# viniciusvidal2/slam-sensor-fusion

Hardware: AMD Instinct MI355X
Metric: scans_per_s_200k_scan_vs_10M_map (higher is better)
Workload: dtype f32 points / f64 accumulation

## Files before the change

slam_sensor_fusion_amd/csrc/sf_nn.hpp:

```cpp
#pragma once
#include "sf_common.hpp"

namespace sf {

#ifdef SF_PHASE_TRACE
constexpr int PH_SLOTS = 16, PH_SHARDS = 64;
struct PhaseClock {
    unsigned long long t;
    unsigned acc[PH_SLOTS];
    __device__ __forceinline__ void start() { for (int i = 0; i < PH_SLOTS; ++i) acc[i] = 0; t = __builtin_amdgcn_s_memtime(); }
    __device__ __forceinline__ void mark(int i) { const unsigned long long n = __builtin_amdgcn_s_memtime(); acc[i] += (unsigned)(n - t); t = n; }
    __device__ __forceinline__ void count(int i, unsigned v) { acc[i] += v; }
};
#define SF_PH(pc, i) do { if (pc) (pc)->mark(i); } while (0)
#define SF_PHC(pc, i, v) do { if (pc) (pc)->count(i, v); } while (0)
#else
struct PhaseClock {};
#define SF_PH(pc, i) do { } while (0)
#define SF_PHC(pc, i, v) do { } while (0)
#endif

struct NNHit {
    float d2;
    int j;
    float px, py, pz;
    float lb2;
};

__device__ __forceinline__ float l2_simple(float qx, float qy, float qz, float px, float py, float pz)
{
    float dx = qx - px, dy = qy - py, dz = qz - pz;
    float r = __fmul_rn(dx, dx);
    r = __fadd_rn(r, __fmul_rn(dy, dy));
    r = __fadd_rn(r, __fmul_rn(dz, dz));
    return r;
}

__device__ __forceinline__ bool window_accepts(const SfWindow &w, float px, float py, float pz)
{
    if (w.kind == 1) return l2_simple(w.c[0], w.c[1], w.c[2], px, py, pz) < w.r2;
    if (w.kind == 2) {
        double d0 = (double)px - w.oc[0], d1 = (double)py - w.oc[1], d2 = (double)pz - w.oc[2];
        bool ok = true;
#pragma unroll
        for (int k = 0; k < 3; ++k) {
            double proj = __dadd_rn(__dadd_rn(__dmul_rn(d0, w.oR[k]), __dmul_rn(d1, w.oR[3 + k])), __dmul_rn(d2, w.oR[6 + k]));
            ok = ok && (fabs(proj) <= w.ohalf[k]);
        }
        return ok;
    }
    return true;
}

__device__ __forceinline__ float window_gap(const SfWindow &w, float qx, float qy, float qz)
{
    if (w.kind == 1) {
        const float dx = qx - w.c[0], dy = qy - w.c[1], dz = qz - w.c[2];
        return fmaxf(sqrtf(dx * dx + dy * dy + dz * dz) * 0.9995f - sqrtf(w.r2) * 1.0005f - 1.0e-4f, 0.0f);
    }
    if (w.kind == 2) {
        const double d0 = (double)qx - w.oc[0], d1 = (double)qy - w.oc[1], d2 = (double)qz - w.oc[2];
        double out = 0.0;
#pragma unroll
        for (int k = 0; k < 3; ++k) {
            const double proj = d0 * w.oR[k] + d1 * w.oR[3 + k] + d2 * w.oR[6 + k];
            const double n2 = w.oR[k] * w.oR[k] + w.oR[3 + k] * w.oR[3 + k] + w.oR[6 + k] * w.oR[6 + k];
            const double over = fmax(fabs(proj) - w.ohalf[k], 0.0);
            out = fmax(out, over / sqrt(fmax(n2, 1.0e-30)));
        }
        return fmaxf((float)out * 0.9995f - 1.0e-4f, 0.0f);
    }
    return 0.0f;
}

__device__ __forceinline__ unsigned long long hit_key(float d2, int j) { return ((unsigned long long)__float_as_uint(d2) << 32) | (unsigned long long)(uint32_t)j; }

__device__ __forceinline__ float search_start(float thr) { return thr > 0.0f ? __uint_as_float(__float_as_uint(thr) - 1u) : -1.0f; }

template <bool WINDOW, bool TRACK = false>
__device__ __forceinline__ void consider(const SfWindow &w, float px, float py, float pz, int j, bool valid, float qx, float qy, float qz, NNHit &hit)
{
    const float d2 = l2_simple(qx, qy, qz, px, py, pz);
    const bool take = valid && hit_key(d2, j) < hit_key(hit.d2, hit.j) && (!WINDOW || window_accepts(w, px, py, pz));
    if (TRACK) hit.lb2 = __builtin_amdgcn_fmed3f((valid && j != hit.j) ? d2 : 3.0e38f, hit.d2, hit.lb2);
    if (take) {
        hit.d2 = d2;
        hit.j = j;
        hit.px = px; hit.py = py; hit.pz = pz;
    }
}

#ifndef SF_NN_CLAMPED_LOADS
__device__ __forceinline__ float4 load_point(const SfGrid &g, uint32_t j, bool valid)
{
    typedef unsigned int u4 __attribute__((ext_vector_type(4)));
    const __amdgpu_buffer_rsrc_t rsrc = __builtin_amdgcn_make_buffer_rsrc((void *)g.pts, 0, (int)((uint32_t)g.n * 16u), 0x00020000);
    const u4 v = __builtin_amdgcn_raw_buffer_load_b128(rsrc, valid ? (int)(j * 16u) : -1, 0, 0);
    return make_float4(__uint_as_float(v.x), __uint_as_float(v.y), __uint_as_float(v.z), __uint_as_float(v.w));
}
#endif

template <bool WINDOW, bool TRACK = false>
__device__ __forceinline__ void scan4(const SfGrid &g, const SfWindow &w, uint32_t j, uint32_t b, float qx, float qy, float qz, NNHit &hit)
{
#ifndef SF_NN_CLAMPED_LOADS
    const float4 p0 = load_point(g, j, true), p1 = load_point(g, j + 1, j + 1 < b), p2 = load_point(g, j + 2, j + 2 < b), p3 = load_point(g, j + 3, j + 3 < b);
    consider<WINDOW, TRACK>(w, p0.x, p0.y, p0.z, (int)j, true, qx, qy, qz, hit);
    consider<WINDOW, TRACK>(w, p1.x, p1.y, p1.z, (int)(j + 1), j + 1 < b, qx, qy, qz, hit);
    consider<WINDOW, TRACK>(w, p2.x, p2.y, p2.z, (int)(j + 2), j + 2 < b, qx, qy, qz, hit);
    consider<WINDOW, TRACK>(w, p3.x, p3.y, p3.z, (int)(j + 3), j + 3 < b, qx, qy, qz, hit);
#else
    const uint32_t last = b - 1;
    const uint32_t j1 = min(j + 1, last), j2 = min(j + 2, last), j3 = min(j + 3, last);
    const float4 p0 = g.pts[j], p1 = g.pts[j1], p2 = g.pts[j2], p3 = g.pts[j3];
    consider<WINDOW, TRACK>(w, p0.x, p0.y, p0.z, (int)j, true, qx, qy, qz, hit);
    consider<WINDOW, TRACK>(w, p1.x, p1.y, p1.z, (int)j1, j + 1 < b, qx, qy, qz, hit);
    consider<WINDOW, TRACK>(w, p2.x, p2.y, p2.z, (int)j2, j + 2 < b, qx, qy, qz, hit);
    consider<WINDOW, TRACK>(w, p3.x, p3.y, p3.z, (int)j3, j + 3 < b, qx, qy, qz, hit);
#endif
}

template <bool WINDOW, bool TRACK = false>
__device__ __forceinline__ void scan_range(const SfGrid &g, const SfWindow &w, uint32_t a, uint32_t b, float qx, float qy, float qz, NNHit &hit)
{
    for (uint32_t j = a; j < b; j += 4) scan4<WINDOW, TRACK>(g, w, j, b, qx, qy, qz, hit);
}

__device__ __forceinline__ float min3f(float a, float b, float c) { return fminf(fminf(a, b), c); }

struct __attribute__((packed, aligned(4))) RowBounds { uint32_t s0, s1, s2, s3; };
__device__ __forceinline__ RowBounds load_row_bounds(const SfGrid &g, size_t cell)
{
    return *reinterpret_cast<const RowBounds *>(g.cell_start + cell - 1);
}

template <bool WINDOW>
__device__ __forceinline__ void scan_row(const SfGrid &g, const SfWindow &w, const RowBounds &rb, float gap2yz, float gxm2, float gxp2, bool xm, bool xp, float qx,
                                         float qy, float qz, NNHit &hit)
{
    scan_range<WINDOW>(g, w, rb.s1, rb.s2, qx, qy, qz, hit);
    if (xm && (gap2yz + gxm2) * 0.998f < hit.d2) scan_range<WINDOW>(g, w, rb.s0, rb.s1, qx, qy, qz, hit);
    if (xp && (gap2yz + gxp2) * 0.998f < hit.d2) scan_range<WINDOW>(g, w, rb.s2, rb.s3, qx, qy, qz, hit);
}

__device__ __forceinline__ float safe_gap(float gap, float eps) { return fmaxf(gap - eps, 0.0f); }

__device__ __forceinline__ float cell_gap(float gc, int c, int cq)
{
    if (c == cq) return 0.0f;
    float d = c < cq ? gc - (float)(c + 1) : (float)c - gc;
    return d > 0.0f ? d : 0.0f;
}

template <bool WINDOW>
__device__ __forceinline__ void nn_rings(const SfGrid &g, const SfWindow &w, float qx, float qy, float qz, int R_first, NNHit &hit)
{
    const float gx = (qx - g.org[0]) * g.inv_h, gy = (qy - g.org[1]) * g.inv_h, gz = (qz - g.org[2]) * g.inv_h;
    const int nx = g.dim[0], ny = g.dim[1], nz = g.dim[2];
    const int cx = (int)fminf(fmaxf(floorf(gx), 0.0f), (float)(nx - 1));
    const int cy = (int)fminf(fmaxf(floorf(gy), 0.0f), (float)(ny - 1));
    const int cz = (int)fminf(fmaxf(floorf(gz), 0.0f), (float)(nz - 1));
    const float h = g.h;
    const int rcap = max(nx, max(ny, nz));

    for (int R = R_first; R <= rcap; ++R) {
        {
            const int x0 = max(cx - R, 0), x1 = min(cx + R, nx - 1);
            const int y0 = max(cy - R, 0), y1 = min(cy + R, ny - 1);
            const int z0 = max(cz - R, 0), z1 = min(cz + R, nz - 1);
            if (R == 1) {
                constexpr uint32_t OYP = 0u | (2u << 2) | (1u << 4) | (1u << 6) | (0u << 8) | (2u << 10) | (0u << 12) | (2u << 14);
                constexpr uint32_t OZP = 1u | (1u << 2) | (0u << 4) | (2u << 6) | (0u << 8) | (0u << 10) | (2u << 12) | (2u << 14);
                const float fx = gx - (float)cx, fy = gy - (float)cy, fz = gz - (float)cz;
                const float ge = g.gap_eps;
                const float gxm = safe_gap(fx * h, ge), gxp = safe_gap((1.0f - fx) * h, ge);
                const float gym = safe_gap(fy * h, ge), gyp = safe_gap((1.0f - fy) * h, ge);
                const float gzm = safe_gap(fz * h, ge), gzp = safe_gap((1.0f - fz) * h, ge);
                const float gxm2 = gxm * gxm, gxp2 = gxp * gxp;
                const bool xm = cx > 0, xp = cx < nx - 1;
                auto row_gap2 = [&](int k) -> float {
                    const int dy = (int)((OYP >> (2 * k)) & 3u) - 1, dz = (int)((OZP >> (2 * k)) & 3u) - 1;
                    const float ry = dy < 0 ? gym : (dy > 0 ? gyp : 0.0f);
                    const float rz = dz < 0 ? gzm : (dz > 0 ? gzp : 0.0f);
                    return ry * ry + rz * rz;
                };
                auto row_cell = [&](int k) -> size_t {
                    const int dy = (int)((OYP >> (2 * k)) & 3u) - 1, dz = (int)((OZP >> (2 * k)) & 3u) - 1;
                    return ((size_t)(cz + dz) * ny + (cy + dy)) * nx + cx;
                };
                {
                    const RowBounds rb = load_row_bounds(g, ((size_t)cz * ny + cy) * nx + cx);
                    scan_row<WINDOW>(g, w, rb, 0.0f, gxm2, gxp2, xm, xp, qx, qy, qz, hit);
                }
                uint32_t mask = 0;
#pragma unroll
                for (int k = 0; k < 8; ++k) {
                    const int dy = (int)((OYP >> (2 * k)) & 3u) - 1, dz = (int)((OZP >> (2 * k)) & 3u) - 1;
                    const bool inside = (unsigned)(cy + dy) < (unsigned)ny && (unsigned)(cz + dz) < (unsigned)nz;
                    if (inside && row_gap2(k) * 0.998f < hit.d2) mask |= 1u << k;
                }
                int k = -1;
                RowBounds cur = {0, 0, 0, 0};
                if (mask) {
                    k = __ffs((int)mask) - 1;
                    mask &= mask - 1;
                    cur = load_row_bounds(g, row_cell(k));
                }
                while (k >= 0) {
                    int k1 = -1;
                    RowBounds nxt = cur;
                    while (mask) {
                        const int kk = __ffs((int)mask) - 1;
                        mask &= mask - 1;
                        if (row_gap2(kk) * 0.998f < hit.d2) {
                            k1 = kk;
                            nxt = load_row_bounds(g, row_cell(kk));
                            break;
                        }
                    }
                    const float g2 = row_gap2(k);
                    if (g2 * 0.998f < hit.d2) scan_row<WINDOW>(g, w, cur, g2, gxm2, gxp2, xm, xp, qx, qy, qz, hit);
                    k = k1;
                    cur = nxt;
                }
            } else {
                for (int z = z0; z <= z1; ++z) {
                    const float rz = safe_gap(cell_gap(gz, z, cz) * h, g.gap_eps);
                    for (int y = y0; y <= y1; ++y) {
                        const float ry = safe_gap(cell_gap(gy, y, cy) * h, g.gap_eps);
                        if ((ry * ry + rz * rz) * 0.998f >= hit.d2) continue;
                        const size_t row = ((size_t)z * ny + y) * nx;
                        scan_range<WINDOW>(g, w, g.cell_start[row + x0], g.cell_start[row + x1 + 1], qx, qy, qz, hit);
                    }
                }
            }
        }
        float m = 3.0e38f;
        if (cx - R > 0) m = fminf(m, (gx - (float)(cx - R)) * h);
        if (cx + R < nx - 1) m = fminf(m, ((float)(cx + R + 1) - gx) * h);
        if (cy - R > 0) m = fminf(m, (gy - (float)(cy - R)) * h);
        if (cy + R < ny - 1) m = fminf(m, ((float)(cy + R + 1) - gy) * h);
        if (cz - R > 0) m = fminf(m, (gz - (float)(cz - R)) * h);
        if (cz + R < nz - 1) m = fminf(m, ((float)(cz + R + 1) - gz) * h);
        if (m >= 3.0e38f) break;
        const float mm = safe_gap(m, g.gap_eps) * 0.999f;
        if (hit.d2 <= mm * mm) break;
    }
}

template <bool WINDOW>
__device__ __forceinline__ NNHit nn_search(const SfGrid &g, const SfWindow &w, float qx, float qy, float qz, float thr)
{
    NNHit hit;
    hit.d2 = search_start(thr);
    hit.j = -1;
    hit.px = hit.py = hit.pz = 0.0f;
    hit.lb2 = 0.0f;
    if (!(isfinite(qx) && isfinite(qy) && isfinite(qz)) || g.n == 0) return hit;
    if (WINDOW) {
        const float gap = window_gap(w, qx, qy, qz);
        if (gap * gap > thr) return hit;
    }
    nn_rings<WINDOW>(g, w, qx, qy, qz, 1, hit);
    return hit;
}

struct WaveNN {
    unsigned long long best[64];
    uint32_t lb2[64];
    float4 q[64];
    RowBounds rb0[64];
    float gap[6][64];
    unsigned long long cell0[64];
    uint16_t task[64 * 11];
};

__device__ __forceinline__ unsigned long long pack_hit(float d2, int j) { return ((unsigned long long)__float_as_uint(d2) << 32) | (unsigned long long)(uint32_t)j; }

struct QueryGeo {
    int cx, cy, cz;
    float gxm2, gxp2;
    float gym, gyp, gzm, gzp;
};

__device__ __forceinline__ QueryGeo query_geo(const SfGrid &g, float qx, float qy, float qz)
{
    QueryGeo G;
    const float gx = (qx - g.org[0]) * g.inv_h, gy = (qy - g.org[1]) * g.inv_h, gz = (qz - g.org[2]) * g.inv_h;
    G.cx = (int)fminf(fmaxf(floorf(gx), 0.0f), (float)(g.dim[0] - 1));
    G.cy = (int)fminf(fmaxf(floorf(gy), 0.0f), (float)(g.dim[1] - 1));
    G.cz = (int)fminf(fmaxf(floorf(gz), 0.0f), (float)(g.dim[2] - 1));
    const float h = g.h;
    const float fx = gx - (float)G.cx, fy = gy - (float)G.cy, fz = gz - (float)G.cz;
    const float ge = g.gap_eps;
    const float gxm = safe_gap(fx * h, ge), gxp = safe_gap((1.0f - fx) * h, ge);
    G.gxm2 = G.cx > 0 ? gxm * gxm : 3.0e38f;
    G.gxp2 = G.cx < g.dim[0] - 1 ? gxp * gxp : 3.0e38f;
    G.gym = safe_gap(fy * h, ge);
    G.gyp = safe_gap((1.0f - fy) * h, ge);
    G.gzm = safe_gap(fz * h, ge);
    G.gzp = safe_gap((1.0f - fz) * h, ge);
    return G;
}

__device__ __forceinline__ int row_dy(int k) { return (int)((0x8858u >> (2 * k)) & 3u) - 1; }
__device__ __forceinline__ int row_dz(int k) { return (int)((0xa085u >> (2 * k)) & 3u) - 1; }

__device__ __forceinline__ float row_gap2(const QueryGeo &G, int k)
{
    const int dy = row_dy(k), dz = row_dz(k);
    const float ry = dy < 0 ? G.gym : (dy > 0 ? G.gyp : 0.0f);
    const float rz = dz < 0 ? G.gzm : (dz > 0 ? G.gzp : 0.0f);
    return ry * ry + rz * rz;
}

template <bool WINDOW, bool COOP = false>
__device__ __forceinline__ NNHit nn_search_wave(const SfGrid &g, const SfWindow &w, bool valid, float qx, float qy, float qz, float thr, WaveNN *ws, NNHit seed = NNHit{0.0f, -1, 0.0f, 0.0f, 0.0f, 0.0f},
                                               PhaseClock *pc = nullptr)
{
    const int lane = (int)__lane_id();
    const int nx = g.dim[0], ny = g.dim[1], nz = g.dim[2];
    NNHit hit;
    hit.d2 = search_start(thr);
    hit.j = -1;
    hit.px = hit.py = hit.pz = 0.0f;
    hit.lb2 = 3.0e38f;
    valid = valid && isfinite(qx) && isfinite(qy) && isfinite(qz) && g.n > 0;
    if (WINDOW && valid) {
        const float gap = window_gap(w, qx, qy, qz);
        if (gap * gap > thr) {
            hit.lb2 = gap * gap;
            valid = false;
        }
    }
    if (valid) {
        const float ox = fmaxf(fmaxf(g.org[0] - qx, qx - (g.org[0] + (float)nx * g.h)), 0.0f);
        const float oy = fmaxf(fmaxf(g.org[1] - qy, qy - (g.org[1] + (float)ny * g.h)), 0.0f);
        const float oz = fmaxf(fmaxf(g.org[2] - qz, qz - (g.org[2] + (float)nz * g.h)), 0.0f);
        const float gap = fmaxf(sqrtf(ox * ox + oy * oy + oz * oz) * 0.9995f - 1.0e-3f, 0.0f);
        if (gap * gap > thr) {
            hit.lb2 = gap * gap;
            valid = false;
        }
    }
    if (valid && seed.j >= 0 && seed.d2 < thr) { hit.d2 = seed.d2; hit.j = seed.j; hit.px = seed.px; hit.py = seed.py; hit.pz = seed.pz; }
    uint32_t mask = 0;
#ifdef SF_PHASE_TRACE
    QueryGeo G{};
    RowBounds rb0{0, 0, 0, 0};
    if (valid) {
        G = query_geo(g, qx, qy, qz);
        rb0 = load_row_bounds(g, ((size_t)G.cz * ny + G.cy) * nx + G.cx);
        ws->rb0[lane] = rb0;
    }
    SF_PH(pc, 1);
    if (valid && rb0.s1 < rb0.s2) scan4<WINDOW, true>(g, w, rb0.s1, rb0.s2, qx, qy, qz, hit);
    SF_PH(pc, 2);
    if (valid) {
#else
    if (valid) {
        const QueryGeo G = query_geo(g, qx, qy, qz);
        const RowBounds rb0 = load_row_bounds(g, ((size_t)G.cz * ny + G.cy) * nx + G.cx);
        ws->rb0[lane] = rb0;
        if (rb0.s1 < rb0.s2) scan4<WINDOW, true>(g, w, rb0.s1, rb0.s2, qx, qy, qz, hit);
#endif
        if (rb0.s1 + 4 < rb0.s2) {
            if (hit.d2 > 0.0f) mask |= 1u << 10;
            else hit.lb2 = 0.0f;
        }
        if (rb0.s0 < rb0.s1) {
            if (G.gxm2 * 0.998f < hit.d2) mask |= 1u;
            else hit.lb2 = fminf(hit.lb2, G.gxm2);
        }
        if (rb0.s2 < rb0.s3) {
            if (G.gxp2 * 0.998f < hit.d2) mask |= 2u;
            else hit.lb2 = fminf(hit.lb2, G.gxp2);
        }
#pragma unroll
        for (int k = 0; k < 8; ++k) {
            const bool inside = (unsigned)(G.cy + row_dy(k)) < (unsigned)ny && (unsigned)(G.cz + row_dz(k)) < (unsigned)nz;
            const float gap2 = row_gap2(G, k);
            if (inside) {
                if (gap2 * 0.998f < hit.d2) mask |= 4u << k;
                else hit.lb2 = fminf(hit.lb2, gap2);
            }
        }
        if (mask) {
            ws->gap[0][lane] = G.gxm2; ws->gap[1][lane] = G.gxp2;
            ws->gap[2][lane] = G.gym; ws->gap[3][lane] = G.gyp; ws->gap[4][lane] = G.gzm; ws->gap[5][lane] = G.gzp;
            ws->cell0[lane] = ((unsigned long long)G.cz * (unsigned long long)ny + (unsigned long long)G.cy) * (unsigned long long)nx + (unsigned long long)G.cx;
        }
    }
    ws->best[lane] = pack_hit(hit.d2, hit.j);
    ws->lb2[lane] = __float_as_uint(hit.lb2);
    ws->q[lane] = make_float4(qx, qy, qz, 0.0f);
    int total = 0;
#pragma unroll
    for (int t = 0; t < 11; ++t) {
        const bool has = (mask >> t) & 1u;
        const unsigned long long bal = __ballot(has);
        const int rank = (int)__builtin_amdgcn_mbcnt_hi((uint32_t)(bal >> 32), __builtin_amdgcn_mbcnt_lo((uint32_t)bal, 0u));
        if (has) ws->task[total + rank] = (uint16_t)((lane << 4) | t);
        total += __popcll(bal);
    }
    __builtin_amdgcn_fence(__ATOMIC_ACQ_REL, "wavefront");
    __builtin_amdgcn_wave_barrier();
    SF_PH(pc, 3);
    SF_PHC(pc, 11, (unsigned)total);
#ifdef SF_PHASE_TRACE
    unsigned lane_trips = 0, lane_cands = 0;
#endif
    for (int i0 = 0; i0 < total; i0 += 64) {
        SF_PHC(pc, 9, 1u);
        const int idx = i0 + lane;
#ifdef SF_PHASE_TRACE
        unsigned my_trips = 0;
#endif
        if (idx < total) {
            const uint32_t e = ws->task[idx];
            const int owner = (int)(e >> 4), t = (int)(e & 15u);
            const float4 Q = ws->q[owner];
            QueryGeo G;
            G.cx = G.cy = G.cz = 0;
            G.gxm2 = ws->gap[0][owner]; G.gxp2 = ws->gap[1][owner];
            G.gym = ws->gap[2][owner]; G.gyp = ws->gap[3][owner]; G.gzm = ws->gap[4][owner]; G.gzp = ws->gap[5][owner];
            const unsigned long long start = __atomic_load_n(&ws->best[owner], __ATOMIC_RELAXED);
            const float cur = __uint_as_float((uint32_t)(start >> 32));
            const bool own_row = t < 2 || t == 10;
            const float g2 = own_row ? (t == 0 ? G.gxm2 : (t == 1 ? G.gxp2 : 0.0f)) : row_gap2(G, t - 2);
            float bound = g2;
            if (g2 * 0.998f < cur) {
                uint32_t a, b;
                bound = 3.0e38f;
                if (own_row) {
                    const RowBounds rb = ws->rb0[owner];
                    a = t == 0 ? rb.s0 : (t == 1 ? rb.s2 : rb.s1 + 4);
                    b = t == 0 ? rb.s1 : (t == 1 ? rb.s3 : rb.s2);
                } else {
                    const long long step = ((long long)row_dz(t - 2) * ny + row_dy(t - 2)) * nx;
                    const RowBounds rb = load_row_bounds(g, (size_t)((long long)ws->cell0[owner] + step));
                    const bool xm = (g2 + G.gxm2) * 0.998f < cur, xp = (g2 + G.gxp2) * 0.998f < cur;
                    a = xm ? rb.s0 : rb.s1;
                    b = xp ? rb.s3 : rb.s2;
                    if (!xm && rb.s0 < rb.s1) bound = g2 + G.gxm2;
                    if (!xp && rb.s2 < rb.s3) bound = fminf(bound, g2 + G.gxp2);
                }
                NNHit h;
                h.d2 = cur;
                h.j = (int)(uint32_t)start;
                h.px = h.py = h.pz = 0.0f;
                h.lb2 = 3.0e38f;
                scan_range<WINDOW, true>(g, w, a, b, Q.x, Q.y, Q.z, h);
#ifdef SF_PHASE_TRACE
                my_trips = (b - a + 3u) / 4u; lane_cands += b - a; lane_trips += my_trips;
#endif
                bound = fminf(bound, h.lb2);
                const unsigned long long mine = pack_hit(h.d2, h.j);
                if (mine != start) {
                    const unsigned long long old = atomicMin(&ws->best[owner], mine);
                    bound = fminf(bound, __uint_as_float((uint32_t)((old > mine ? old : mine) >> 32)));
                }
            }
            atomicMin(&ws->lb2[owner], __float_as_uint(bound));
        }
#ifdef SF_PHASE_TRACE
        { unsigned m = my_trips; for (int o = 32; o > 0; o >>= 1) m = max(m, (unsigned)__shfl_xor((int)m, o)); SF_PHC(pc, 10, m); }
#endif
    }
    __builtin_amdgcn_fence(__ATOMIC_ACQ_REL, "wavefront");
    __builtin_amdgcn_wave_barrier();
    SF_PH(pc, 4);
#ifdef SF_PHASE_TRACE
    { unsigned m = lane_trips, c = lane_cands; for (int o = 32; o > 0; o >>= 1) { m += (unsigned)__shfl_xor((int)m, o); c += (unsigned)__shfl_xor((int)c, o); } SF_PHC(pc, 12, m); SF_PHC(pc, 13, c); }
#endif
    bool more = false;
    if (valid) {
        const unsigned long long m = ws->best[lane];
        const int j = (int)(uint32_t)m;
        hit.lb2 = __uint_as_float(ws->lb2[lane]);
        if (j != hit.j) {
            const float4 p = g.pts[j];
            hit.d2 = __uint_as_float((uint32_t)(m >> 32));
            hit.j = j;
            hit.px = p.x; hit.py = p.y; hit.pz = p.z;
        }
        const float gx = (qx - g.org[0]) * g.inv_h, gy = (qy - g.org[1]) * g.inv_h, gz = (qz - g.org[2]) * g.inv_h;
        const int cx = (int)fminf(fmaxf(floorf(gx), 0.0f), (float)(nx - 1));
        const int cy = (int)fminf(fmaxf(floorf(gy), 0.0f), (float)(ny - 1));
        const int cz = (int)fminf(fmaxf(floorf(gz), 0.0f), (float)(nz - 1));
        const float h = g.h;
        float mface = 3.0e38f;
        if (cx - 1 > 0) mface = fminf(mface, (gx - (float)(cx - 1)) * h);
        if (cx + 1 < nx - 1) mface = fminf(mface, ((float)(cx + 2) - gx) * h);
        if (cy - 1 > 0) mface = fminf(mface, (gy - (float)(cy - 1)) * h);
        if (cy + 1 < ny - 1) mface = fminf(mface, ((float)(cy + 2) - gy) * h);
        if (cz - 1 > 0) mface = fminf(mface, (gz - (float)(cz - 1)) * h);
        if (cz + 1 < nz - 1) mface = fminf(mface, ((float)(cz + 2) - gz) * h);
        const float mm = safe_gap(mface, g.gap_eps) * 0.999f;
        if (mface < 3.0e38f) {
            hit.lb2 = fminf(hit.lb2, mm * mm);
            more = !(hit.d2 <= mm * mm);
        }
        if (!COOP && more) {
            nn_rings<WINDOW>(g, w, qx, qy, qz, 2, hit);
            hit.lb2 = 0.0f;
        }
    }
    SF_PH(pc, 5);
    if (!COOP) return hit;
    unsigned long long unres = __ballot(more);
    const int rcap = max(nx, max(ny, nz));
    for (int R = 2; unres != 0ull && R <= rcap; ++R) {
        {
            const int rank = (int)__builtin_amdgcn_mbcnt_hi((uint32_t)(unres >> 32), __builtin_amdgcn_mbcnt_lo((uint32_t)unres, 0u));
            if (more) {
                ws->task[rank] = (uint16_t)lane;
                ws->best[lane] = pack_hit(hit.d2, hit.j);
            }
        }
        __builtin_amdgcn_fence(__ATOMIC_ACQ_REL, "wavefront");
        __builtin_amdgcn_wave_barrier();
        const int side = 2 * R + 1, nrows = side * side, total = __popcll(unres) * nrows;
        const float h = g.h, ge = g.gap_eps;
        for (int idx = lane; idx < total; idx += 64) {
            const int u = idx / nrows, r = idx - u * nrows;
            const int owner = (int)ws->task[u];
            const int dyi = r / side - R, dzi = r - (r / side) * side - R;
            const float4 Q = ws->q[owner];
            const float gx = (Q.x - g.org[0]) * g.inv_h, gy = (Q.y - g.org[1]) * g.inv_h, gz = (Q.z - g.org[2]) * g.inv_h;
            const int cx = (int)fminf(fmaxf(floorf(gx), 0.0f), (float)(nx - 1));
            const int cy = (int)fminf(fmaxf(floorf(gy), 0.0f), (float)(ny - 1));
            const int cz = (int)fminf(fmaxf(floorf(gz), 0.0f), (float)(nz - 1));
            const int y = cy + dyi, z = cz + dzi;
            if ((unsigned)y >= (unsigned)ny || (unsigned)z >= (unsigned)nz) continue;
            const float ry = safe_gap(cell_gap(gy, y, cy) * h, ge), rz = safe_gap(cell_gap(gz, z, cz) * h, ge);
            const float g2 = ry * ry + rz * rz;
            const unsigned long long start = __atomic_load_n(&ws->best[owner], __ATOMIC_RELAXED);
            const float cur = __uint_as_float((uint32_t)(start >> 32));
            if (g2 * 0.998f >= cur) continue;
            NNHit t;
            t.d2 = cur;
            t.j = (int)(uint32_t)start;
            t.px = t.py = t.pz = 0.0f;
            t.lb2 = 0.0f;
            const size_t row = ((size_t)z * ny + y) * nx;
            const bool inner = abs(dyi) < R && abs(dzi) < R;
            if (!inner) {
                const int x0 = max(cx - R, 0), x1 = min(cx + R, nx - 1);
                scan_range<WINDOW>(g, w, g.cell_start[row + x0], g.cell_start[row + x1 + 1], Q.x, Q.y, Q.z, t);
            } else {
                if (cx - R >= 0) {
                    const float gl = safe_gap((gx - (float)(cx - R + 1)) * h, ge);
                    if ((g2 + gl * gl) * 0.998f < t.d2) scan_range<WINDOW>(g, w, g.cell_start[row + cx - R], g.cell_start[row + cx - R + 1], Q.x, Q.y, Q.z, t);
                }
                if (cx + R <= nx - 1) {
                    const float gr = safe_gap(((float)(cx + R) - gx) * h, ge);
                    if ((g2 + gr * gr) * 0.998f < t.d2) scan_range<WINDOW>(g, w, g.cell_start[row + cx + R], g.cell_start[row + cx + R + 1], Q.x, Q.y, Q.z, t);
                }
            }
            const unsigned long long mine = pack_hit(t.d2, t.j);
            if (mine != start) atomicMin(&ws->best[owner], mine);
        }
        __builtin_amdgcn_fence(__ATOMIC_ACQ_REL, "wavefront");
        __builtin_amdgcn_wave_barrier();
        if (more) {
            const unsigned long long m = ws->best[lane];
            const int j = (int)(uint32_t)m;
            if (j != hit.j) {
                const float4 p = g.pts[j];
                hit.d2 = __uint_as_float((uint32_t)(m >> 32));
                hit.j = j;
                hit.px = p.x; hit.py = p.y; hit.pz = p.z;
            }
            hit.lb2 = 0.0f;
            const float gx = (qx - g.org[0]) * g.inv_h, gy = (qy - g.org[1]) * g.inv_h, gz = (qz - g.org[2]) * g.inv_h;
            const int cx = (int)fminf(fmaxf(floorf(gx), 0.0f), (float)(nx - 1));
            const int cy = (int)fminf(fmaxf(floorf(gy), 0.0f), (float)(ny - 1));
            const int cz = (int)fminf(fmaxf(floorf(gz), 0.0f), (float)(nz - 1));
            float mface = 3.0e38f;
            if (cx - R > 0) mface = fminf(mface, (gx - (float)(cx - R)) * h);
            if (cx + R < nx - 1) mface = fminf(mface, ((float)(cx + R + 1) - gx) * h);
            if (cy - R > 0) mface = fminf(mface, (gy - (float)(cy - R)) * h);
            if (cy + R < ny - 1) mface = fminf(mface, ((float)(cy + R + 1) - gy) * h);
            if (cz - R > 0) mface = fminf(mface, (gz - (float)(cz - R)) * h);
            if (cz + R < nz - 1) mface = fminf(mface, ((float)(cz + R + 1) - gz) * h);
            const float mm = safe_gap(mface, ge) * 0.999f;
            more = mface < 3.0e38f && !(hit.d2 <= mm * mm);
        }
        unres = __ballot(more);
    }
    return hit;
}

}
```

Baseline: 18450.

## Deal neighbor-row candidate points across wave lanes via prefix-scan load balancing

For the non-window path, the per-task row scans are replaced by a wave-wide load-balanced scheme. A DPP prefix sum over the task lengths sets each task's offset, a mark array with a max-scan maps each flat candidate index back to its owning task, and every lane then evaluates NN_DEAL_K points per round, updating best and lower-bound entries with LDS atomics. This removes divergence caused by unequal row lengths, where one long row held the whole wave. In exchange it adds extra scans, bpermutes, LDS traffic and atomics per candidate, and it gives up the early pruning that scan_range does as the best distance shrinks.

```diff
diff --git a/slam_sensor_fusion_amd/csrc/sf_nn.hpp b/slam_sensor_fusion_amd/csrc/sf_nn.hpp
--- a/slam_sensor_fusion_amd/csrc/sf_nn.hpp
+++ b/slam_sensor_fusion_amd/csrc/sf_nn.hpp
@@ -265,14 +265,19 @@
     return hit;
 }
 
+#ifndef SF_NN_DEAL_K
+#define SF_NN_DEAL_K 2
+#endif
+constexpr int NN_DEAL_K = SF_NN_DEAL_K;
 struct WaveNN {
     unsigned long long best[64];
     uint32_t lb2[64];
     float4 q[64];
     RowBounds rb0[64];
-    float gap[6][64];
+    float gap[5][64];
     unsigned long long cell0[64];
     uint16_t task[64 * 11];
+    alignas(4) uint8_t mark[64 * NN_DEAL_K];
 };
 
 __device__ __forceinline__ unsigned long long pack_hit(float d2, int j) { return ((unsigned long long)__float_as_uint(d2) << 32) | (unsigned long long)(uint32_t)j; }
@@ -314,6 +319,71 @@
     return ry * ry + rz * rz;
 }
 
+template <bool MAX>
+__device__ __forceinline__ uint32_t wave_incl_scan(uint32_t v)
+{
+    auto op = [](uint32_t a, uint32_t b) { return MAX ? max(a, b) : a + b; };
+    v = op(v, (uint32_t)__builtin_amdgcn_update_dpp(0, (int)v, 0x111, 0xf, 0xf, false));
+    v = op(v, (uint32_t)__builtin_amdgcn_update_dpp(0, (int)v, 0x112, 0xf, 0xf, false));
+    v = op(v, (uint32_t)__builtin_amdgcn_update_dpp(0, (int)v, 0x114, 0xf, 0xf, false));
+    v = op(v, (uint32_t)__builtin_amdgcn_update_dpp(0, (int)v, 0x118, 0xf, 0xf, false));
+    v = op(v, (uint32_t)__builtin_amdgcn_update_dpp(0, (int)v, 0x142, 0xa, 0xf, false));
+    v = op(v, (uint32_t)__builtin_amdgcn_update_dpp(0, (int)v, 0x143, 0xc, 0xf, false));
+    return v;
+}
+
+__device__ __forceinline__ void wave_sync()
+{
+    __builtin_amdgcn_fence(__ATOMIC_ACQ_REL, "wavefront");
+    __builtin_amdgcn_wave_barrier();
+}
+
+struct RoundTask {
+    int owner;
+    bool live;
+    uint32_t a, b;
+    float bound;
+    float4 Q;
+    unsigned long long start;
+};
+
+__device__ __forceinline__ RoundTask round_task(const SfGrid &g, WaveNN *ws, uint32_t e)
+{
+    const int nx = g.dim[0], ny = g.dim[1];
+    RoundTask T;
+    T.owner = (int)(e >> 4);
+    const int owner = T.owner, t = (int)(e & 15u);
+    T.Q = ws->q[owner];
+    QueryGeo G;
+    G.cx = G.cy = G.cz = 0;
+    G.gxm2 = T.Q.w; G.gxp2 = ws->gap[0][owner];
+    G.gym = ws->gap[1][owner]; G.gyp = ws->gap[2][owner]; G.gzm = ws->gap[3][owner]; G.gzp = ws->gap[4][owner];
+    T.start = __atomic_load_n(&ws->best[owner], __ATOMIC_RELAXED);
+    const float cur = __uint_as_float((uint32_t)(T.start >> 32));
+    const bool own_row = t < 2 || t == 10;
+    const float g2 = own_row ? (t == 0 ? G.gxm2 : (t == 1 ? G.gxp2 : 0.0f)) : row_gap2(G, t - 2);
+    T.bound = g2;
+    T.a = T.b = 0;
+    T.live = g2 * 0.998f < cur;
+    if (T.live) {
+        T.bound = 3.0e38f;
+        if (own_row) {
+            const RowBounds rb = ws->rb0[owner];
+            T.a = t == 0 ? rb.s0 : (t == 1 ? rb.s2 : rb.s1 + 4);
+            T.b = t == 0 ? rb.s1 : (t == 1 ? rb.s3 : rb.s2);
+        } else {
+            const long long step = ((long long)row_dz(t - 2) * ny + row_dy(t - 2)) * nx;
+            const RowBounds rb = load_row_bounds(g, (size_t)((long long)ws->cell0[owner] + step));
+            const bool xm = (g2 + G.gxm2) * 0.998f < cur, xp = (g2 + G.gxp2) * 0.998f < cur;
+            T.a = xm ? rb.s0 : rb.s1;
+            T.b = xp ? rb.s3 : rb.s2;
+            if (!xm && rb.s0 < rb.s1) T.bound = g2 + G.gxm2;
+            if (!xp && rb.s2 < rb.s3) T.bound = fminf(T.bound, g2 + G.gxp2);
+        }
+    }
+    return T;
+}
+
 template <bool WINDOW, bool COOP = false>
 __device__ __forceinline__ NNHit nn_search_wave(const SfGrid &g, const SfWindow &w, bool valid, float qx, float qy, float qz, float thr, WaveNN *ws, NNHit seed = NNHit{0.0f, -1, 0.0f, 0.0f, 0.0f, 0.0f},
                                                PhaseClock *pc = nullptr)
@@ -345,6 +415,7 @@
     }
     if (valid && seed.j >= 0 && seed.d2 < thr) { hit.d2 = seed.d2; hit.j = seed.j; hit.px = seed.px; hit.py = seed.py; hit.pz = seed.pz; }
     uint32_t mask = 0;
+    float q_gxm2 = 0.0f;
 #ifdef SF_PHASE_TRACE
     QueryGeo G{};
     RowBounds rb0{0, 0, 0, 0};
@@ -386,14 +457,15 @@
             }
         }
         if (mask) {
-            ws->gap[0][lane] = G.gxm2; ws->gap[1][lane] = G.gxp2;
-            ws->gap[2][lane] = G.gym; ws->gap[3][lane] = G.gyp; ws->gap[4][lane] = G.gzm; ws->gap[5][lane] = G.gzp;
+            q_gxm2 = G.gxm2;
+            ws->gap[0][lane] = G.gxp2;
+            ws->gap[1][lane] = G.gym; ws->gap[2][lane] = G.gyp; ws->gap[3][lane] = G.gzm; ws->gap[4][lane] = G.gzp;
             ws->cell0[lane] = ((unsigned long long)G.cz * (unsigned long long)ny + (unsigned long long)G.cy) * (unsigned long long)nx + (unsigned long long)G.cx;
         }
     }
     ws->best[lane] = pack_hit(hit.d2, hit.j);
     ws->lb2[lane] = __float_as_uint(hit.lb2);
-    ws->q[lane] = make_float4(qx, qy, qz, 0.0f);
+    ws->q[lane] = make_float4(qx, qy, qz, q_gxm2);
     int total = 0;
 #pragma unroll
     for (int t = 0; t < 11; ++t) {
@@ -413,59 +485,100 @@
     for (int i0 = 0; i0 < total; i0 += 64) {
         SF_PHC(pc, 9, 1u);
         const int idx = i0 + lane;
+        if constexpr (WINDOW) {
 #ifdef SF_PHASE_TRACE
-        unsigned my_trips = 0;
-#endif
-        if (idx < total) {
-            const uint32_t e = ws->task[idx];
-            const int owner = (int)(e >> 4), t = (int)(e & 15u);
-            const float4 Q = ws->q[owner];
-            QueryGeo G;
-            G.cx = G.cy = G.cz = 0;
-            G.gxm2 = ws->gap[0][owner]; G.gxp2 = ws->gap[1][owner];
-            G.gym = ws->gap[2][owner]; G.gyp = ws->gap[3][owner]; G.gzm = ws->gap[4][owner]; G.gzp = ws->gap[5][owner];
-            const unsigned long long start = __atomic_load_n(&ws->best[owner], __ATOMIC_RELAXED);
-            const float cur = __uint_as_float((uint32_t)(start >> 32));
-            const bool own_row = t < 2 || t == 10;
-            const float g2 = own_row ? (t == 0 ? G.gxm2 : (t == 1 ? G.gxp2 : 0.0f)) : row_gap2(G, t - 2);
-            float bound = g2;
-            if (g2 * 0.998f < cur) {
-                uint32_t a, b;
-                bound = 3.0e38f;
-                if (own_row) {
-                    const RowBounds rb = ws->rb0[owner];
-                    a = t == 0 ? rb.s0 : (t == 1 ? rb.s2 : rb.s1 + 4);
-                    b = t == 0 ? rb.s1 : (t == 1 ? rb.s3 : rb.s2);
-                } else {
-                    const long long step = ((long long)row_dz(t - 2) * ny + row_dy(t - 2)) * nx;
-                    const RowBounds rb = load_row_bounds(g, (size_t)((long long)ws->cell0[owner] + step));
-                    const bool xm = (g2 + G.gxm2) * 0.998f < cur, xp = (g2 + G.gxp2) * 0.998f < cur;
-                    a = xm ? rb.s0 : rb.s1;
-                    b = xp ? rb.s3 : rb.s2;
-                    if (!xm && rb.s0 < rb.s1) bound = g2 + G.gxm2;
-                    if (!xp && rb.s2 < rb.s3) bound = fminf(bound, g2 + G.gxp2);
-                }
-                NNHit h;
-                h.d2 = cur;
-                h.j = (int)(uint32_t)start;
-                h.px = h.py = h.pz = 0.0f;
-                h.lb2 = 3.0e38f;
-                scan_range<WINDOW, true>(g, w, a, b, Q.x, Q.y, Q.z, h);
+            unsigned my_trips = 0;
+#endif
+            if (idx < total) {
+                const RoundTask T = round_task(g, ws, ws->task[idx]);
+                float bound = T.bound;
+                if (T.live) {
+                    NNHit h;
+                    h.d2 = __uint_as_float((uint32_t)(T.start >> 32));
+                    h.j = (int)(uint32_t)T.start;
+                    h.px = h.py = h.pz = 0.0f;
+                    h.lb2 = 3.0e38f;
+                    scan_range<WINDOW, true>(g, w, T.a, T.b, T.Q.x, T.Q.y, T.Q.z, h);
 #ifdef SF_PHASE_TRACE
-                my_trips = (b - a + 3u) / 4u; lane_cands += b - a; lane_trips += my_trips;
-#endif
-                bound = fminf(bound, h.lb2);
-                const unsigned long long mine = pack_hit(h.d2, h.j);
-                if (mine != start) {
-                    const unsigned long long old = atomicMin(&ws->best[owner], mine);
-                    bound = fminf(bound, __uint_as_float((uint32_t)((old > mine ? old : mine) >> 32)));
-                }
+                    my_trips = (T.b - T.a + 3u) / 4u; lane_cands += T.b - T.a; lane_trips += my_trips;
+#endif
+                    bound = fminf(bound, h.lb2);
+                    const unsigned long long mine = pack_hit(h.d2, h.j);
+                    if (mine != T.start) {
+                        const unsigned long long old = atomicMin(&ws->best[T.owner], mine);
+                        bound = fminf(bound, __uint_as_float((uint32_t)((old > mine ? old : mine) >> 32)));
+                    }
+                }
+                atomicMin(&ws->lb2[T.owner], __float_as_uint(bound));
             }
-            atomicMin(&ws->lb2[owner], __float_as_uint(bound));
-        }
 #ifdef SF_PHASE_TRACE
-        { unsigned m = my_trips; for (int o = 32; o > 0; o >>= 1) m = max(m, (unsigned)__shfl_xor((int)m, o)); SF_PHC(pc, 10, m); }
-#endif
+            { unsigned m = my_trips; for (int o = 32; o > 0; o >>= 1) m = max(m, (unsigned)__shfl_xor((int)m, o)); SF_PHC(pc, 10, m); }
+#endif
+        } else {
+            uint32_t a = 0, len = 0;
+            int owner = 0;
+            if (idx < total) {
+                const RoundTask T = round_task(g, ws, ws->task[idx]);
+                owner = T.owner;
+                if (T.live) { a = T.a; len = T.b - T.a; }
+                atomicMin(&ws->lb2[owner], __float_as_uint(T.bound));
+            }
+            const uint32_t incl = wave_incl_scan<false>(len);
+            const uint32_t off = incl - len;
+            const uint32_t tot = (uint32_t)__builtin_amdgcn_readlane((int)incl, 63);
+            const uint32_t base = a - off;
+            SF_PHC(pc, 13, tot);
+            uint32_t carry = 0;
+            for (uint32_t c0 = 0; c0 < tot; c0 += 64u * NN_DEAL_K) {
+                SF_PHC(pc, 10, 1u);
+                for (int i = lane; i < 16 * NN_DEAL_K; i += 64) reinterpret_cast<uint32_t *>(ws->mark)[i] = 0u;
+                __builtin_amdgcn_wave_barrier();
+                if (len != 0u && off - c0 < 64u * NN_DEAL_K && off >= c0) ws->mark[off - c0] = (uint8_t)(lane + 1);
+                wave_sync();
+                uint32_t src[NN_DEAL_K];
+#pragma unroll
+                for (int k = 0; k < NN_DEAL_K; ++k) src[k] = wave_incl_scan<true>((uint32_t)ws->mark[64 * k + lane]);
+#pragma unroll
+                for (int k = 0; k < NN_DEAL_K; ++k) {
+                    src[k] = max(src[k], carry);
+                    carry = (uint32_t)__builtin_amdgcn_readlane((int)src[k], 63);
+                }
+                wave_sync();
+                SF_PHC(pc, 12, (unsigned)__popcll(__ballot(c0 + (uint32_t)lane < tot)));
+                uint32_t j[NN_DEAL_K];
+                int ow[NN_DEAL_K];
+                float4 p[NN_DEAL_K], Q[NN_DEAL_K];
+                unsigned long long cur[NN_DEAL_K];
+#pragma unroll
+                for (int k = 0; k < NN_DEAL_K; ++k) {
+                    const uint32_t s = c0 + 64u * (uint32_t)k + (uint32_t)lane;
+                    const int from = (int)((src[k] - 1u) & 63u) << 2;
+                    j[k] = (uint32_t)__builtin_amdgcn_ds_bpermute(from, (int)base) + s;
+                    ow[k] = __builtin_amdgcn_ds_bpermute(from, owner);
+                    p[k] = load_point(g, j[k], s < tot);
+                }
+#pragma unroll
+                for (int k = 0; k < NN_DEAL_K; ++k) {
+                    Q[k] = ws->q[ow[k]];
+                    cur[k] = __atomic_load_n(&ws->best[ow[k]], __ATOMIC_RELAXED);
+                }
+#pragma unroll
+                for (int k = 0; k < NN_DEAL_K; ++k) {
+                    const bool live = c0 + 64u * (uint32_t)k + (uint32_t)lane < tot;
+                    const float d2 = l2_simple(Q[k].x, Q[k].y, Q[k].z, p[k].x, p[k].y, p[k].z);
+                    const unsigned long long mine = pack_hit(d2, (int)j[k]);
+                    if (live && mine != cur[k]) {
+                        uint32_t lose = __float_as_uint(d2);
+                        if (mine < cur[k]) {
+                            const unsigned long long old = atomicMin(&ws->best[ow[k]], mine);
+                            lose = (uint32_t)((old > mine ? old : mine) >> 32);
+                        }
+                        atomicMin(&ws->lb2[ow[k]], lose);
+                    }
+                }
+            }
+            wave_sync();
+        }
     }
     __builtin_amdgcn_fence(__ATOMIC_ACQ_REL, "wavefront");
     __builtin_amdgcn_wave_barrier();
```

New measurement: 19220, median of 6. 1.04x the previous value.
